# sunhui-3D/3D-PointCloudReconstruction

Hardware: AMD Instinct MI355X
Metric: Chamfer3D fwd+bwd point-pairs/sec @ B=32 N=M=1024; EMD iters/sec (higher is better)
Workload: dtype f32; 1 GPU; Chamfer3D fwd+bwd (+loss sums, +RCCL all-reduce of every step's loss when N>1); batch_per_gpu=32, n_points=1024, m_points=1024, global_batch=32, parallelism=dp1 (batch-sharded), launch=hipgraph (20 steps per graph; N>1 adds each step's all-reduce to the same graph)

## Files before the change

3d-pointcloudreconstruction_amd/csrc/chamfer_filt.hip:

```cpp
#include <type_traits>

#include "pcm_common.h"
#include "pcm_internal.h"
#include "chamfer_loss.h"

namespace {
using namespace pcm_loss;

constexpr float kFiltU16 = 9.5367431640625e-07f;

#ifdef PCM_STAMPS
constexpr int kStampSlots = 1 << 16;
__device__ unsigned long long g_pcm_stamps[kStampSlots * 8];
#define PCM_STAMP(i)                                                                           \
    do {                                                                                       \
        if (threadIdx.x == 0 && blockIdx.x < kStampSlots)                                      \
            g_pcm_stamps[blockIdx.x * 8 + (i)] = __builtin_amdgcn_s_memrealtime();            \
    } while (0)
#define PCM_STAMP2(i)                                                                          \
    do {                                                                                       \
        if (threadIdx.x == 0 && blockIdx.x < kStampSlots / 2)                                  \
            g_pcm_stamps[(kStampSlots / 2 + blockIdx.x) * 8 + (i)] = __builtin_amdgcn_s_memrealtime(); \
    } while (0)
#else
// ... 363 lines not shown
                    if (resident) {
#pragma unroll
                        for (int k = 0; k < CP; ++k) {
                            const int kk = slot(min(k0 + k, nt - 1));
                            const pcm_f4 t4 = sT[kk];
                            tx[k] = t4.x;
                            ty[k] = t4.y;
                            tz[k] = t4.z;
                        }
                    } else {
#pragma unroll
                        for (int k = 0; k < CP; ++k) {
                            const int kk = min(k0 + k, nt - 1);
                            tx[k] = pcm_ld(T + pcm_at(LT, kk, 0));
                            ty[k] = pcm_ld(T + pcm_at(LT, kk, 1));
                            tz[k] = pcm_ld(T + pcm_at(LT, kk, 2));
                        }
                    }
#pragma unroll
                    for (int k = 0; k < CP; ++k) {
                        const float d = pcm_sqd(tx[k] - x, ty[k] - y, tz[k] - z);
                        const bool take = (d < hd) & (k0 + k < nt);
                        hd = take ? d : hd;
                        hk = take ? k0 + k : hk;
                    }
                } else if (part == 0) {
                    unsigned plan = 0;
                    const float thr = fb + e2;
#pragma unroll
                    for (int w = 0; w < W; ++w)
                        plan |= !(vs[w] > thr) ? (1u << (W + w)) : (!(vb[w] > thr) ? (1u << w) : 0u);
                    sPlan[s] = plan;
                    sList[atomicAdd(&sNList, 1)] = s;
                }
            }
            sHD[part][s] = hd;
            sHK[part][s] = hk;
        }
        __syncthreads();
        PCM_STAMP(5);

        const int nl = sNList;
        if (resident) {
            static_assert(C <= 64 && 64 % C == 0 && 64 % W == 0 && (TILE / C) % W == 0,
                          "whole chunks per step; wave w owns the chunks c = w mod W");
            constexpr int kCps = 64 / C;
            unsigned long long wpat = 0;
#pragma unroll
            for (int i = 0; i < 64; i += W) wpat |= 1ull << i;
            const int nch = (nt + C - 1) / C;
            for (int e = wave; e < nl; e += W) {
                const int s = __builtin_amdgcn_readfirstlane(sList[e]);
                const unsigned plan = __builtin_amdgcn_readfirstlane(sPlan[s]);
                int one[W];
#pragma unroll
                for (int w = 0; w < W; ++w) one[w] = __builtin_amdgcn_readfirstlane(sChunk[w][s]);
                float x = rx[0], y = ry[0], z = rz[0];
#pragma unroll
                for (int qq = 1; qq < QPT; ++qq)
                    if ((s >> 6) == qq) { x = rx[qq]; y = ry[qq]; z = rz[qq]; }
                x = __int_as_float(__builtin_amdgcn_readlane(__float_as_int(x), s & 63));
                y = __int_as_float(__builtin_amdgcn_readlane(__float_as_int(y), s & 63));
                z = __int_as_float(__builtin_amdgcn_readlane(__float_as_int(z), s & 63));
                float bd = PCM_INF;
                int bk = 0x7fffffff;
                for (int c0 = 0; c0 < nch; c0 += 64) {
                    unsigned long long M = 0;
#pragma unroll
                    for (int w = 0; w < W; ++w) {
                        if ((plan >> (W + w)) & 1u) M |= wpat << w;
                        else if (((plan >> w) & 1u) && one[w] >= c0 && one[w] < c0 + 64) M |= 1ull << (one[w] - c0);
                    }
                    if (nch - c0 < 64) M &= (1ull << (nch - c0)) - 1ull;
                    while (M) {
                        int ch[kCps];
#pragma unroll
                        for (int j = 0; j < kCps; ++j) {
                            ch[j] = M ? c0 + __builtin_ctzll(M) : -1;
                            M &= M - 1ull;
                        }
                        int c = ch[0];
#pragma unroll
                        for (int j = 1; j < kCps; ++j)
                            if (lane / C == j) c = ch[j];
                        const int k = c * C + (lane & (C - 1));
                        const int sk = slot(min(max(k, 0), nt - 1));
                        const pcm_f4 t4 = sT[sk];
                        const float d = pcm_sqd(t4.x - x, t4.y - y, t4.z - z);
                        if (c >= 0 && k < nt) pcm_lexmin(bd, bk, d, k);
                    }
                }
                pcm_wave_lexmin(bd, bk);
                if (lane == 0) {
                    sD[s] = bd;
                    sK[s] = bk;
                }
            }
            if (nl > 0) __syncthreads();
        }
        for (int e0 = 0; e0 < (resident ? 0 : nl); e0 += kTB) {
            float qx[kTB], qy[kTB], qz[kTB], bd[kTB];
            int bk[kTB];
#pragma unroll
            for (int j = 0; j < kTB; ++j) {
                const int s = sList[min(e0 + j, nl - 1)];
                float x = rx[0], y = ry[0], z = rz[0];
#pragma unroll
                for (int qq = 1; qq < QPT; ++qq)
                    if ((s >> 6) == qq) { x = rx[qq]; y = ry[qq]; z = rz[qq]; }
                qx[j] = __shfl(x, s & 63, 64);
                qy[j] = __shfl(y, s & 63, 64);
                qz[j] = __shfl(z, s & 63, 64);
                bd[j] = PCM_INF;
                bk[j] = 0x7fffffff;
            }
            auto visit = [&](int k, float x, float y, float z) {
#pragma unroll
                for (int j = 0; j < kTB; ++j) {
                    const float d = pcm_sqd(x - qx[j], y - qy[j], z - qz[j]);
                    pcm_lexmin(bd[j], bk[j], d, k);
                }
            };
            {
                constexpr int U = 8;
                for (int k0 = tid; k0 < nt; k0 += U * NT) {
                    float tx[U], ty[U], tz[U];
#pragma unroll
                    for (int u = 0; u < U; ++u) {
                        const int k = min(k0 + u * NT, nt - 1);
                        tx[u] = pcm_ld(T + pcm_at(LT, k, 0));
                        ty[u] = pcm_ld(T + pcm_at(LT, k, 1));
                        tz[u] = pcm_ld(T + pcm_at(LT, k, 2));
                    }
#pragma unroll
                    for (int u = 0; u < U; ++u)
                        if (k0 + u * NT < nt) visit(k0 + u * NT, tx[u], ty[u], tz[u]);
                }
            }
#pragma unroll
            for (int j = 0; j < kTB; ++j) {
#pragma unroll
                for (int o = 32; o > 0; o >>= 1) {
                    const float od = __shfl_xor(bd[j], o, 64);
                    const int ok = __shfl_xor(bk[j], o, 64);
                    pcm_lexmin(bd[j], bk[j], od, ok);
                }
            }
            if (lane == 0) {
#pragma unroll
                for (int j = 0; j < kTB; ++j) {
                    sTD[j * W + wave] = bd[j];
                    sTK[j * W + wave] = bk[j];
                }
            }
            __syncthreads();
            if (tid < kTB && e0 + tid < nl) {
                float d = sTD[tid * W];
                int k = sTK[tid * W];
                for (int w = 1; w < W; ++w) {
                    const float dv = sTD[tid * W + w];
                    const int kv = sTK[tid * W + w];
                    pcm_lexmin(d, k, dv, kv);
                }
                const int s = sList[e0 + tid];
                sD[s] = d;
                sK[s] = k;
            }
            __syncthreads();
        }
        PCM_STAMP(6);
        int kg = 0;
        if (tid < QW && qbase + tid < nq) {
            float d;
            int k;
            if (proven) {
                d = sHD[0][tid];
                k = sHK[0][tid];
#pragma unroll
                for (int p = 1; p < PARTS; ++p) pcm_lexmin(d, k, sHD[p][tid], sHK[p][tid]);
            } else {
                d = sD[tid];
                k = sK[tid];
            }
            my_d = d;
            out_st<kSc1>(D + qbase + tid, d);
            out_st<kSc1>(I + qbase + tid, (int32_t)k);
            if (Gr) __hip_atomic_store(Gr + qbase + tid, tag | (unsigned)k, __ATOMIC_RELAXED, __HIP_MEMORY_SCOPE_AGENT);
            if (Gr4 && !g4x)
                __hip_atomic_store(Gr4 + qbase + tid, gtag4 | (unsigned)k, __ATOMIC_RELAXED, __HIP_MEMORY_SCOPE_AGENT);
            if (kown) *kown = k;
            kg = k;
        }
        if (Gr4 && g4x && tid < QW) {
            const unsigned v = gtag4 | (unsigned)kg;
            const int src = (lane & 15) * 4;
            pcm_u32x4 g;
            g.x = (unsigned)__shfl((int)v, src, 64);
            g.y = (unsigned)__shfl((int)v, src + 1, 64);
            g.z = (unsigned)__shfl((int)v, src + 2, 64);
            g.w = (unsigned)__shfl((int)v, src + 3, 64);
            const int q = qbase + (tid & ~63) + src;
            if (lane < 16 && q < nq) {
                if (q + 3 < nq) {
                    pcm_st_sc1_x4(Gr4 + q, g);
                } else {
                    __hip_atomic_store(Gr4 + q, g.x, __ATOMIC_RELAXED, __HIP_MEMORY_SCOPE_AGENT);
                    if (q + 1 < nq) __hip_atomic_store(Gr4 + q + 1, g.y, __ATOMIC_RELAXED, __HIP_MEMORY_SCOPE_AGENT);
                    if (q + 2 < nq) __hip_atomic_store(Gr4 + q + 2, g.z, __ATOMIC_RELAXED, __HIP_MEMORY_SCOPE_AGENT);
                }
            }
        }
    } else {
        for (int s = tid; s < QW; s += NT) {
            const int qi = qbase + s;
            if (qi >= nq) continue;
            float d;
            int idx;
            pcm_ref_nn_scan(pcm_ld(Q + pcm_at(LQ, qi, 0)), pcm_ld(Q + pcm_at(LQ, qi, 1)),
                            pcm_ld(Q + pcm_at(LQ, qi, 2)), T, nt, d, idx, LT);
            my_d = d;
            out_st<kSc1>(D + qi, d);
            out_st<kSc1>(I + qi, (int32_t)idx);
            if (Gr) __hip_atomic_store(Gr + qi, tag | (unsigned)idx, __ATOMIC_RELAXED, __HIP_MEMORY_SCOPE_AGENT);
            if (Gr4) __hip_atomic_store(Gr4 + qi, gtag4 | (unsigned)idx, __ATOMIC_RELAXED, __HIP_MEMORY_SCOPE_AGENT);
            if (kown) *kown = idx;
        }
    }
    return my_d;
}

constexpr float kFiltU80 = 4.76837158203125e-06f;
constexpr int kMfmaQW = 256, kMfmaNT = 512, kMfmaTile = 1024;
struct MfmaLds {
    static constexpr int kA = kMfmaTile * 48;
    static constexpr int kZ = (3 * 48 + 16) * 16;
    static constexpr int kQB = kMfmaQW * 48;
    static constexpr int kScan = kA + kZ + kQB;
    static constexpr int kTail = 3 * kMfmaTile * 4 + 3 * 4 * kMfmaQW * 4;
    static constexpr int kBytes = kScan > kTail ? kScan : kTail;
};
typedef __bf16 pcm_bf16x8 __attribute__((ext_vector_type(8)));

typedef __bf16 pcm_bf16x2 __attribute__((ext_vector_type(2)));
__device__ __forceinline__ unsigned cvt_bf16x2(float a, float b) {
    return __builtin_bit_cast(unsigned, __builtin_convertvector((pcm_f2){a, b}, pcm_bf16x2));
}
__device__ __forceinline__ float bf_lo(unsigned v) { return __uint_as_float(v << 16); }
__device__ __forceinline__ float bf_hi(unsigned v) { return __uint_as_float(v & 0xffff0000u); }
template <int HL, int HH>
__device__ __forceinline__ unsigned bf_pair(unsigned lo, unsigned hi) {
    constexpr unsigned sel = (HL ? 0x0302u : 0x0100u) | ((HH ? 0x0706u : 0x0504u) << 16);
    return __builtin_amdgcn_perm(hi, lo, sel);
}
[[maybe_unused]] __device__ __forceinline__ void split3x2(float a, float b, unsigned &H, unsigned &M, unsigned &L) {
    H = cvt_bf16x2(a, b);
    const float ra = a - bf_lo(H), rb = b - bf_hi(H);
    M = cvt_bf16x2(ra, rb);
    L = cvt_bf16x2(ra - bf_lo(M), rb - bf_hi(M));
}
[[maybe_unused]] __device__ __forceinline__ int mslot(int p) { return (p & ~63) | ((p + 4 * ((p >> 6) & 7)) & 63); }

template <bool k32>
__device__ __forceinline__ void mfma_fold_step(float &b, float &s, int &c, float bo, float so, int co) {
    auto swap = [](unsigned &x, unsigned &y) {
        if constexpr (k32) {
            const auto r = __builtin_amdgcn_permlane32_swap(x, y, false, false);
            x = r[0];
            y = r[1];
        } else {
            const auto r = __builtin_amdgcn_permlane16_swap(x, y, false, false);
            x = r[0];
            y = r[1];
        }
    };
    unsigned b0 = __float_as_uint(b), b1 = __float_as_uint(bo), s0 = __float_as_uint(s), s1 = __float_as_uint(so);
    unsigned c0 = (unsigned)c, c1 = (unsigned)co;
    swap(b0, b1);
    swap(s0, s1);
    swap(c0, c1);
    const float fb0 = __uint_as_float(b0), fb1 = __uint_as_float(b1);
    const bool better = (fb1 < fb0) | ((fb1 == fb0) & ((int)c1 < (int)c0));
    s = __builtin_fminf(__builtin_fminf(__uint_as_float(s0), __uint_as_float(s1)), better ? fb0 : fb1);
    b = better ? fb1 : fb0;
    c = better ? (int)c1 : (int)c0;
}

template <bool kSc1>
__device__ __forceinline__ float filt_forward_mfma(const float *__restrict__ Q, const float *__restrict__ T, int nq,
                                                   int nt, int qbase, float *__restrict__ D, int32_t *__restrict__ I,
                                                   unsigned char *arena, unsigned long long *__restrict__ Gr = nullptr,
                                                   unsigned long long tag = 0, PcmLay LQ = PcmLay{3, 1},
                                                   PcmLay LT = PcmLay{3, 1}, int *kown = nullptr) {
    constexpr int QW = kMfmaQW, NT = kMfmaNT, W = NT / 64, TILE = kMfmaTile, QPT = QW / 64;
    constexpr int kPer = TILE / NT;
    static_assert(NT == 2 * QW && QPT == 4, "thread = (query slot, part of 2); wave w holds query copy w mod 4");
    uint4 *sA = reinterpret_cast<uint4 *>(arena);
    uint4 *sZ = reinterpret_cast<uint4 *>(arena + MfmaLds::kA);
    uint4 *sQB = reinterpret_cast<uint4 *>(arena + MfmaLds::kA + MfmaLds::kZ);
    auto rowslot = [](int p, int j) { return 48 * (p >> 4) + 16 * j + (p & 15); };
    float(*sT)[TILE] = reinterpret_cast<float(*)[TILE]>(arena);
    float(*sPB)[QW] = reinterpret_cast<float(*)[QW]>(arena + 3 * TILE * 4);
    float(*sPS)[QW] = reinterpret_cast<float(*)[QW]>(arena + 3 * TILE * 4 + 4 * QW * 4);
    int(*sPC)[QW] = reinterpret_cast<int(*)[QW]>(arena + 3 * TILE * 4 + 8 * QW * 4);
    __shared__ float sD[QW];
    __shared__ int sK[QW];
    __shared__ unsigned sPlan[QW];
    __shared__ float sHD[2][QW];
    __shared__ int sHK[2][QW];
    __shared__ float sRmax[W];
    __shared__ int sList[QW];
    __shared__ int sNList;
    __shared__ int sNFm[W];

    const int tid = threadIdx.x, lane = tid & 63;
    const int wave = __builtin_amdgcn_readfirstlane(tid >> 6);

    float rx[QPT], ry[QPT], rz[QPT];
#pragma unroll
    for (int qq = 0; qq < QPT; ++qq) {
        const int qc = min(qbase + qq * 64 + lane, nq - 1);
        rx[qq] = pcm_ld(Q + pcm_at(LQ, qc, 0));
        ry[qq] = pcm_ld(Q + pcm_at(LQ, qc, 1));
        rz[qq] = pcm_ld(Q + pcm_at(LQ, qc, 2));
    }
    float tv[kPer][3];
#pragma unroll
    for (int r = 0; r < kPer; ++r) {
        const int p = min(tid + r * NT, nt - 1);
#pragma unroll
        for (int d = 0; d < 3; ++d) tv[r][d] = pcm_ld(T + pcm_at(LT, p, d));
    }
    bool nonfinite = false;
    float cx = 0.f, cy = 0.f, cz = 0.f;
    int qcnt = 0;
#pragma unroll
    for (int qq = 0; qq < QPT; ++qq) {
        if (qbase + qq * 64 + lane < nq) {
            nonfinite |= !(pcm_finite(rx[qq]) && pcm_finite(ry[qq]) && pcm_finite(rz[qq]));
            cx += rx[qq];
            cy += ry[qq];
            cz += rz[qq];
            ++qcnt;
        }
    }
    if (tid == 0) sNList = 0;
    const float cn = (float)wave_sum_dpp(qcnt);
    const float c0 = wave_sum_dpp(cx) / cn, c1 = wave_sum_dpp(cy) / cn, c2 = wave_sum_dpp(cz) / cn;
    PCM_STAMP(1);
#ifdef PCM_STAMPS
    if (tid == 0 && blockIdx.x < 4096)
        g_pcm_stamps[(8192 + blockIdx.x) * 8 + 1] = __builtin_amdgcn_s_memtime();
#endif

    float qx = rx[0], qy = ry[0], qz = rz[0];
#pragma unroll
    for (int qq = 1; qq < QPT; ++qq)
        if ((wave & (QPT - 1)) == qq) { qx = rx[qq]; qy = ry[qq]; qz = rz[qq]; }
    const float qxc = qx - c0, qyc = qy - c1, qzc = qz - c2;
    {
        unsigned H01, M01, L01, H2, M2, L2;
        split3x2(qxc, qyc, H01, M01, L01);
        split3x2(qzc, 0.f, H2, M2, L2);
        const unsigned one2 = 0x3f803f80u, one0 = 0x00003f80u;
        const int row = tid & (QW - 1);
        if (wave < QPT) {
            sQB[rowslot(row, 0)] = make_uint4(bf_pair<0, 0>(H01, M01), bf_pair<0, 0>(H01, L01), bf_pair<0, 0>(H01, M01),
                                              bf_pair<1, 1>(H01, M01));
            sQB[rowslot(row, 1)] = make_uint4(bf_pair<1, 1>(H01, L01), bf_pair<1, 1>(H01, M01), bf_pair<0, 0>(H2, M2),
                                              bf_pair<0, 0>(H2, L2));
        } else {
            sQB[rowslot(row, 2)] = make_uint4(bf_pair<0, 0>(H2, M2), one2, one0, 0u);
            if (row < MfmaLds::kZ / 16) sZ[row] = make_uint4(0u, 0u, 0u, 0u);
        }
    }
    const int ntp = (nt + 63) & ~63;
    float rt2 = 0.f;
    uint4 rows[kPer][3];
#pragma unroll
    for (int r = 0; r < kPer; ++r) {
        nonfinite |= !(pcm_finite(tv[r][0]) && pcm_finite(tv[r][1]) && pcm_finite(tv[r][2]));
        const float x = tv[r][0] - c0, y = tv[r][1] - c1, z = tv[r][2] - c2;
        const float w = __builtin_fmaf(z, z, __builtin_fmaf(y, y, x * x));
        unsigned H01, M01, L01, H23, M23, L23;
        split3x2(-2.f * x, -2.f * y, H01, M01, L01);
        split3x2(-2.f * z, w, H23, M23, L23);
        rt2 = __builtin_fmaxf(rt2, __builtin_fmaxf(w, bf_hi(H23)));
        const bool pad = tid + r * NT >= nt;
        rows[r][0] = make_uint4(bf_pair<0, 0>(H01, H01), bf_pair<0, 0>(M01, H01), bf_pair<0, 0>(L01, M01),
                                bf_pair<1, 1>(H01, H01));
        rows[r][1] = make_uint4(bf_pair<1, 1>(M01, H01), bf_pair<1, 1>(L01, M01), bf_pair<0, 0>(H23, H23),
                                bf_pair<0, 0>(M23, H23));
        rows[r][2] = make_uint4(bf_pair<0, 0>(L23, M23), bf_pair<1, 1>(H23, M23), L23 >> 16, 0u);
        if (pad) {
            rows[r][0] = make_uint4(0u, 0u, 0u, 0u);
            rows[r][1] = make_uint4(0u, 0u, 0u, 0u);
            rows[r][2] = make_uint4(0u, 0x00007f80u, 0u, 0u);
        }
    }
#pragma unroll
    for (int r = 0; r < kPer; ++r) {
        const int p = tid + r * NT;
        if (p < ntp) {
            sA[rowslot(p, 0)] = rows[r][0];
            sA[rowslot(p, 1)] = rows[r][1];
            sA[rowslot(p, 2)] = rows[r][2];
        }
    }
    {
        const float v = pcm_wave_max_f32(rt2);
        if (lane == 0) sRmax[wave] = v;
    }
    __syncthreads();
    PCM_STAMP(2);

    const int quarter = wave >> 1, half = wave & 1;
    const int g = lane >> 4, col = lane & 15;
    constexpr int QT = QW / 2 / 16;
    const uint4 *pq = g < 3 ? sQB + 48 * half * QT + lane : sZ + col;
    const uint4 *pa = g < 3 ? sA + lane : sZ + col;
    const int tstep = g < 3 ? 48 : 0;
    pcm_bf16x8 bq[QT];
#pragma unroll
    for (int qt = 0; qt < QT; ++qt) bq[qt] = __builtin_bit_cast(pcm_bf16x8, pq[qt * tstep]);
    float best[QT], sec[QT];
    int bchunk[QT];
#pragma unroll
    for (int qt = 0; qt < QT; ++qt) { best[qt] = PCM_INF; sec[qt] = PCM_INF; bchunk[qt] = 0; }
    const int ngroups = ntp >> 6;
    uint4 an[4];
    auto fetch = [&](int gi, int i) { an[i] = pa[4 * gi * tstep + 48 * i]; };
    if (quarter < ngroups) {
#pragma unroll
        for (int i = 0; i < 4; ++i) fetch(quarter, i);
    }
    for (int gi = quarter; gi < ngroups; gi += 4) {
        const int gn = gi + 4 < ngroups ? gi + 4 : gi;
        float mn[QT];
#pragma unroll
        for (int qt = 0; qt < QT; ++qt) mn[qt] = PCM_INF;
#pragma unroll
        for (int i = 0; i < 4; ++i) {
            const pcm_bf16x8 a = __builtin_bit_cast(pcm_bf16x8, an[i]);
            fetch(gn, i);
            __builtin_amdgcn_sched_barrier(0);
#pragma unroll
            for (int qt = 0; qt < QT; ++qt) {
                const pcm_f4 d = __builtin_amdgcn_mfma_f32_16x16x32_bf16(a, bq[qt], pcm_f4{0.f, 0.f, 0.f, 0.f}, 0, 0, 0);
                mn[qt] = __builtin_fminf(__builtin_fminf(mn[qt], d.x), d.y);
                mn[qt] = __builtin_fminf(__builtin_fminf(mn[qt], d.z), d.w);
            }
            __builtin_amdgcn_sched_group_barrier(0x8, 2, 0);
#pragma unroll
            for (int k = 0; k < QT - 2; ++k) {
                __builtin_amdgcn_sched_group_barrier(0x2, 2, 0);
                __builtin_amdgcn_sched_group_barrier(0x8, 1, 0);
            }
        }
        const int cid = 4 * gi + g;
#pragma unroll
        for (int qt = 0; qt < QT; ++qt) {
            sec[qt] = __builtin_amdgcn_fmed3f(mn[qt], best[qt], sec[qt]);
            if (mn[qt] < best[qt]) { best[qt] = mn[qt]; bchunk[qt] = cid; }
        }
    }
    __syncthreads();
    PCM_STAMP(3);
#pragma unroll
    for (int r = 0; r < kPer; ++r) {
        const int p = tid + r * NT;
        if (p < nt) { sT[0][mslot(p)] = tv[r][0]; sT[1][mslot(p)] = tv[r][1]; sT[2][mslot(p)] = tv[r][2]; }
    }
    static_assert(QT == 8, "two halving steps: 8 query tiles -> 2 per lane");
#pragma unroll
    for (int j = 0; j < 4; ++j)
        mfma_fold_step<true>(best[j], sec[j], bchunk[j], best[j + 4], sec[j + 4], bchunk[j + 4]);
#pragma unroll
    for (int j = 0; j < 2; ++j) {
        mfma_fold_step<false>(best[j], sec[j], bchunk[j], best[j + 2], sec[j + 2], bchunk[j + 2]);
        const int s = half * (QW / 2) + (4 * (g >> 1) + 2 * (g & 1) + j) * 16 + col;
        sPB[quarter][s] = best[j];
        sPS[quarter][s] = sec[j];
        sPC[quarter][s] = bchunk[j];
    }
    const int any_nonfinite = pcm_wg_or(nonfinite, sNFm, W);
    PCM_STAMP(4);

    float my_d = 0.f;
    if (!any_nonfinite) {
        const int s = tid & (QW - 1), part = tid / QW;
        bool proven = false;
        {
            float vb[4], vs[4], vr[W];
            int vc[4];
#pragma unroll
            for (int q = 0; q < 4; ++q) {
                vb[q] = sPB[q][s];
                vs[q] = sPS[q][s];
                vc[q] = sPC[q][s];
            }
#pragma unroll
            for (int w = 0; w < W; ++w) vr[w] = sRmax[w];
            __builtin_amdgcn_sched_barrier(0);
            float fb = vb[0], fs = vs[0];
            int fc = vc[0];
#pragma unroll
            for (int q = 1; q < 4; ++q) {
                const bool better = (vb[q] < fb) | ((vb[q] == fb) & (vc[q] < fc));
                fs = __builtin_fminf(__builtin_fminf(fs, vs[q]), better ? fb : vb[q]);
                fb = better ? vb[q] : fb;
                fc = better ? vc[q] : fc;
            }
            float rmax2 = vr[0];
#pragma unroll
            for (int w = 1; w < W; ++w) rmax2 = __builtin_fmaxf(rmax2, vr[w]);
            const float kAbs = 7.888609052210118e-31f;
            const float qn2 = __builtin_fmaf(qzc, qzc, __builtin_fmaf(qyc, qyc, qxc * qxc));
            const float sq = __builtin_amdgcn_sqrtf(qn2);
            const float rr = __builtin_amdgcn_sqrtf(rmax2) + sq;
            const float eR = kFiltU80 * (rr * rr) * 1.001f + kAbs;
            const float db = __builtin_fmaxf((fb + qn2) * 1.0001f + 2.f * eR, 0.f);
            const float rq = 2.f * sq + __builtin_amdgcn_sqrtf(db);
            const float e2 = 2.f * (kFiltU80 * __builtin_fminf(rr * rr, rq * rq) * 1.001f + kAbs);
            proven = (fs - fb) > e2;
            float hd = PCM_INF;
            int hk = 0x7fffffff;
            if (qbase + s < nq) {
                if (proven) {
                    const int k0 = 64 * (fc >> 2) + 32 * part + 4 * (fc & 3);
                    pcm_f4 tx[2], ty[2], tz[2];
#pragma unroll
                    for (int h = 0; h < 2; ++h) {
                        const int o = mslot(k0 + 16 * h);
                        tx[h] = *reinterpret_cast<const pcm_f4 *>(&sT[0][o]);
                        ty[h] = *reinterpret_cast<const pcm_f4 *>(&sT[1][o]);
                        tz[h] = *reinterpret_cast<const pcm_f4 *>(&sT[2][o]);
                    }
#pragma unroll
                    for (int k = 0; k < 8; ++k) {
                        const int kk = k0 + 16 * (k >> 2) + (k & 3);
                        const float d = pcm_sqd(tx[k >> 2][k & 3] - qx, ty[k >> 2][k & 3] - qy, tz[k >> 2][k & 3] - qz);
                        const bool take = (d < hd) & (kk < nt);
                        hd = take ? d : hd;
                        hk = take ? kk : hk;
                    }
                } else if (part == 0) {
                    const float thr = fb + e2;
                    unsigned plan = 0;
#pragma unroll
                    for (int q = 0; q < 4; ++q) plan |= !(vs[q] > thr) ? (1u << q) : (!(vb[q] > thr) ? (16u << q) : 0u);
                    sPlan[s] = plan;
                    sList[atomicAdd(&sNList, 1)] = s;
                }
            }
            sHD[part][s] = hd;
            sHK[part][s] = hk;
        }
        __syncthreads();
        PCM_STAMP(5);
        const int nl = sNList;
        for (int e = wave; e < nl; e += W) {
            const int sq = __builtin_amdgcn_readfirstlane(sList[e]);
            const unsigned plan = __builtin_amdgcn_readfirstlane(sPlan[sq]);
            float x = rx[0], y = ry[0], z = rz[0];
#pragma unroll
            for (int qq = 1; qq < QPT; ++qq)
                if ((sq >> 6) == qq) { x = rx[qq]; y = ry[qq]; z = rz[qq]; }
            x = __int_as_float(__builtin_amdgcn_readlane(__float_as_int(x), sq & 63));
            y = __int_as_float(__builtin_amdgcn_readlane(__float_as_int(y), sq & 63));
            z = __int_as_float(__builtin_amdgcn_readlane(__float_as_int(z), sq & 63));
            float bd = PCM_INF;
            int bk = 0x7fffffff;
            {
                const int pc = sPC[g][sq];
                const int k = 64 * (pc >> 2) + 16 * (col >> 2) + 4 * (pc & 3) + (col & 3);
                const bool on = ((plan >> (4 + g)) & 1u) && k < nt;
                const int ks = mslot(min(k, nt - 1));
                const float d = pcm_sqd(sT[0][ks] - x, sT[1][ks] - y, sT[2][ks] - z);
                if (on) pcm_lexmin(bd, bk, d, k);
            }
            for (int q = 0; q < 4; ++q) {
                if (!((plan >> q) & 1u)) continue;
                float tx[4], ty[4], tz[4];
                int kk[4];
#pragma unroll
                for (int u = 0; u < 4; ++u) {
                    const int k = 64 * (q + 4 * u) + lane;
                    kk[u] = (q + 4 * u < ngroups && k < nt) ? k : -1;
                    const int ks = mslot(min(max(kk[u], 0), nt - 1));
                    tx[u] = sT[0][ks];
                    ty[u] = sT[1][ks];
                    tz[u] = sT[2][ks];
                }
#pragma unroll
                for (int u = 0; u < 4; ++u) {
                    const float d = pcm_sqd(tx[u] - x, ty[u] - y, tz[u] - z);
                    if (kk[u] >= 0) pcm_lexmin(bd, bk, d, kk[u]);
                }
            }
            pcm_wave_lexmin(bd, bk);
            if (lane == 0) {
                sD[sq] = bd;
                sK[sq] = bk;
            }
        }
        if (nl > 0) __syncthreads();
        PCM_STAMP(6);
#ifdef PCM_STAMPS
        if (tid == 0 && blockIdx.x < 4096) g_pcm_stamps[(8192 + blockIdx.x) * 8 + 6] = __builtin_amdgcn_s_memtime();
        if (tid == NT - 1 && blockIdx.x < kStampSlots) {
            unsigned long long full = 0, single = 0;
            for (int e = 0; e < nl; ++e) {
                const unsigned pl = sPlan[sList[e]];
                full += __popc(pl & 15);
                single += __popc((pl >> 4) & 15);
            }
            g_pcm_stamps[blockIdx.x * 8 + 0] = (unsigned long long)nl | (full << 16) | (single << 40);
        }
#endif
        if (tid < QW && qbase + tid < nq) {
            float d;
            int k;
            if (proven) {
                d = sHD[0][tid];
                k = sHK[0][tid];
                pcm_lexmin(d, k, sHD[1][tid], sHK[1][tid]);
            } else {
                d = sD[tid];
                k = sK[tid];
            }
            my_d = d;
            out_st<kSc1>(D + qbase + tid, d);
            out_st<kSc1>(I + qbase + tid, (int32_t)k);
            if (Gr) __hip_atomic_store(Gr + qbase + tid, tag | (unsigned)k, __ATOMIC_RELAXED, __HIP_MEMORY_SCOPE_AGENT);
            if (kown) *kown = k;
        }
    } else {
        for (int s = tid; s < QW; s += NT) {
            const int qi = qbase + s;
            if (qi >= nq) continue;
            float d;
            int idx;
            pcm_ref_nn_scan(pcm_ld(Q + pcm_at(LQ, qi, 0)), pcm_ld(Q + pcm_at(LQ, qi, 1)),
                            pcm_ld(Q + pcm_at(LQ, qi, 2)), T, nt, d, idx, LT);
            my_d = d;
            out_st<kSc1>(D + qi, d);
            out_st<kSc1>(I + qi, (int32_t)idx);
            if (Gr) __hip_atomic_store(Gr + qi, tag | (unsigned)idx, __ATOMIC_RELAXED, __HIP_MEMORY_SCOPE_AGENT);
            if (kown) *kown = idx;
        }
    }
    return my_d;
}

template <typename TIn, int W, int QPT, int C, int TILE, int kLoss>
__global__ __launch_bounds__(64 * W) __attribute__((amdgpu_waves_per_eu(4))) void chamfer_fwd_filt_kernel(
    const TIn *__restrict__ xyz1, const TIn *__restrict__ xyz2, int b, int n, int m,
    float *__restrict__ dist1, float *__restrict__ dist2, int32_t *__restrict__ idx1,
    int32_t *__restrict__ idx2, int nblk1, int nblk2, float *__restrict__ partials,
    unsigned *__restrict__ ticket, float *__restrict__ mean_out) {
    static_assert(kLoss == 0 || kLoss == 3, "filtered forward publishes granules only");
    static_assert(W <= 16, "sRed holds 16 waves");
    constexpr int QW = 64 * QPT;
    __shared__ float sRed[2][16];

    int nprod = (int)gridDim.x;
    unsigned epoch = 0;
    if constexpr (kLoss == 3) {
        nprod -= 1;
        if ((int)blockIdx.x == nprod) {
            poll_loss(b * nblk1, nprod, b, n, m, reinterpret_cast<const unsigned long long *>(partials), ticket,
                      mean_out);
            return;
        }
        epoch = ticket[kEpochWord] + 1u;
    }
    PCM_STAMP(0);
    int batch, blk;
    bool first;
    pcm_split_bm(pcm_xcd_remap((int)blockIdx.x, nprod), nblk1, nblk2, batch, first, blk);
    const int slot = first ? batch * nblk1 + blk : b * nblk1 + batch * nblk2 + blk;
    const TIn *Q = first ? xyz1 + (size_t)batch * n * 3 : xyz2 + (size_t)batch * m * 3;
    const TIn *T = first ? xyz2 + (size_t)batch * m * 3 : xyz1 + (size_t)batch * n * 3;
    float *D = first ? dist1 + (size_t)batch * n : dist2 + (size_t)batch * m;
    int32_t *I = first ? idx1 + (size_t)batch * n : idx2 + (size_t)batch * m;
    const int nq = first ? n : m, nt = first ? m : n;
    const float my_d = filt_forward<TIn, W, QPT, C, TILE, false>(Q, T, nq, nt, blk * QW, D, I,
                                                                 lds_arena<FiltLds<W, QPT, TILE>::kBytes>());
    if constexpr (kLoss == 3) publish_partial<3>(my_d, slot, partials, ticket, sRed, epoch);
#ifdef PCM_STAMPS
    if (threadIdx.x == 0 && blockIdx.x < kStampSlots)
        g_pcm_stamps[blockIdx.x * 8 + 7] = __builtin_amdgcn_s_memrealtime();
#endif
}

template <int W, int QPT, int C, int TILE, int LAY1, int LAY2>
__global__ __launch_bounds__(64 * W) __attribute__((amdgpu_waves_per_eu(4))) void chamfer_fwd_filt_lay_kernel(
    const float *__restrict__ xyz1, const float *__restrict__ xyz2, int b, int n, int m,
    float *__restrict__ dist1, float *__restrict__ dist2, int32_t *__restrict__ idx1,
    int32_t *__restrict__ idx2, int nblk1, int nblk2) {
    constexpr int QW = 64 * QPT;
    int batch, blk;
    bool first;
    pcm_split_bm(pcm_xcd_remap((int)blockIdx.x, (int)gridDim.x), nblk1, nblk2, batch, first, blk);
    const float *X1 = xyz1 + (size_t)batch * n * 3, *X2 = xyz2 + (size_t)batch * m * 3;
    const PcmLay L1 = LAY1 ? PcmLay{1, n} : PcmLay{3, 1}, L2 = LAY2 ? PcmLay{1, m} : PcmLay{3, 1};
    if (first)
        filt_forward<float, W, QPT, C, TILE, false>(X1, X2, n, m, blk * QW, dist1 + (size_t)batch * n,
                                                   idx1 + (size_t)batch * n, lds_arena<FiltLds<W, QPT, TILE>::kBytes>(),
                                                   nullptr, 0, nullptr, nullptr, L1, L2);
    else
        filt_forward<float, W, QPT, C, TILE, false>(X2, X1, m, n, blk * QW, dist2 + (size_t)batch * m,
                                                   idx2 + (size_t)batch * m, lds_arena<FiltLds<W, QPT, TILE>::kBytes>(),
                                                   nullptr, 0, nullptr, nullptr, L2, L1);
}

constexpr int kGradCap = 1024;
constexpr unsigned kG4TagBits = 21;
constexpr unsigned kG4TagMask = (1u << kG4TagBits) - 1u;
static_assert(kGradCap <= 2048, "a 4-byte granule holds an 11-bit index");
constexpr unsigned kGradWaitSpins = 1u << 16;
constexpr int kGradSlots = 8;
constexpr int kGradSlotsMax = 16;
constexpr int kGradBytes = 2 * kGradCap * 12 + 2 * kGradCap * 4 + 2 * kGradCap * kGradSlots * 2;

__device__ __forceinline__ int32_t ld_sc1(const int32_t *p) {
    return __hip_atomic_load(p, __ATOMIC_RELAXED, __HIP_MEMORY_SCOPE_AGENT);
}
__device__ __forceinline__ float ld_sc1(const float *p) {
    return __hip_atomic_load(p, __ATOMIC_RELAXED, __HIP_MEMORY_SCOPE_AGENT);
}

template <typename GetA, typename GetH>
__device__ __forceinline__ void scatter_sum(float &ax, float &ay, float &az, float sx, float sy, float sz,
                                            GetH h, GetA getA, const uint16_t *tab, int cnt) {
    static_assert(kGradSlots == 8 && kGradSlotsMax == 16, "sorting networks for 8 and 16 ids");
    if (cnt > kGradSlots) {
        int f[16];
        const uint4 r0 = *reinterpret_cast<const uint4 *>(tab);
        const uint4 r1 = *reinterpret_cast<const uint4 *>(tab + 8);
        const unsigned wv[8] = {r0.x, r0.y, r0.z, r0.w, r1.x, r1.y, r1.z, r1.w};
#pragma unroll
        for (int u = 0; u < 16; ++u) {
            const int t = (int)((wv[u >> 1] >> (16 * (u & 1))) & 0xffffu);
            f[u] = u < cnt ? t : 0x7fffffff;
        }
#pragma unroll
        for (int rd = 0; rd < 16; ++rd)
#pragma unroll
            for (int i = rd & 1; i + 1 < 16; i += 2) {
                const int lo = min(f[i], f[i + 1]), hi = max(f[i], f[i + 1]);
                f[i] = lo;
                f[i + 1] = hi;
            }
        for (int u = 0; u < cnt; ++u) {
            float tx, ty, tz;
            getA(f[u], tx, ty, tz);
            const float hu = h(f[u]);
            ax = __fadd_rn(ax, -__fmul_rn(hu, __fsub_rn(tx, sx)));
            ay = __fadd_rn(ay, -__fmul_rn(hu, __fsub_rn(ty, sy)));
            az = __fadd_rn(az, -__fmul_rn(hu, __fsub_rn(tz, sz)));
        }
        return;
    }
    int e[8];
    const uint4 row = *reinterpret_cast<const uint4 *>(tab);
    const unsigned w[4] = {row.x, row.y, row.z, row.w};
#pragma unroll
    for (int u = 0; u < 8; ++u) {
        const int t = (int)((w[u >> 1] >> (16 * (u & 1))) & 0xffffu);
        e[u] = u < cnt ? t : 0x7fffffff;
    }
    auto cas = [&](int i, int j) {
        const int lo = min(e[i], e[j]), hi = max(e[i], e[j]);
        e[i] = lo;
        e[j] = hi;
    };
    cas(0, 1); cas(2, 3); cas(4, 5); cas(6, 7); cas(0, 2); cas(1, 3); cas(4, 6); cas(5, 7); cas(1, 2);
    cas(5, 6); cas(0, 4); cas(3, 7); cas(1, 5); cas(2, 6); cas(1, 4); cas(3, 6); cas(2, 4); cas(3, 5);
    cas(3, 4);
    auto add = [&](float hu, float tx, float ty, float tz) {
        ax = __fadd_rn(ax, -__fmul_rn(hu, __fsub_rn(tx, sx)));
        ay = __fadd_rn(ay, -__fmul_rn(hu, __fsub_rn(ty, sy)));
        az = __fadd_rn(az, -__fmul_rn(hu, __fsub_rn(tz, sz)));
    };
    float gx[4], gy[4], gz[4], gh[4];
#pragma unroll
    for (int u = 0; u < 4; ++u) {
        const int su = u < cnt ? e[u] : 0;
        getA(su, gx[u], gy[u], gz[u]);
        gh[u] = h(su);
    }
#pragma unroll
    for (int u = 0; u < 4; ++u) {
        const bool on = u < cnt;
        const float nx = __fadd_rn(ax, -__fmul_rn(gh[u], __fsub_rn(gx[u], sx)));
        const float ny = __fadd_rn(ay, -__fmul_rn(gh[u], __fsub_rn(gy[u], sy)));
        const float nz = __fadd_rn(az, -__fmul_rn(gh[u], __fsub_rn(gz[u], sz)));
        ax = on ? nx : ax;
        ay = on ? ny : ay;
        az = on ? nz : az;
    }
    for (int u = 4; u < cnt; ++u) {
        float tx, ty, tz;
        getA(e[u], tx, ty, tz);
        add(h(e[u]), tx, ty, tz);
    }
}

constexpr int kBwdSlotsT = 256;
constexpr int kBwdSlotsMax = 2048;

struct PcmRescale {
    const float *gl = nullptr;
    const float *used = nullptr;
    float *next = nullptr;
    float inv1 = 0.f, inv2 = 0.f;
};

__device__ __forceinline__ void slots_task(int task, int ntasks, const float *__restrict__ xyz1,
                                           const float *__restrict__ xyz2, int n, int m,
                                           const float *__restrict__ gd1, const float *__restrict__ gd2,
                                           const int32_t *__restrict__ idx1, const int32_t *__restrict__ idx2,
                                           float *__restrict__ grad1, float *__restrict__ grad2, int nblk1, int nblk2,
                                           int lay1, int lay2, PcmGdStr GS, bool rescale, float rs1, float rs2) {
    constexpr int NT = kBwdSlotsT;
    __shared__ __attribute__((aligned(16))) float sO[3 * kBwdSlotsMax];
    __shared__ __attribute__((aligned(16))) float sG[kBwdSlotsMax];
    __shared__ __attribute__((aligned(16))) int sK[kBwdSlotsMax];
    __shared__ int cnt[NT];
    __shared__ __attribute__((aligned(16))) uint16_t tab[NT * kGradSlotsMax];
    const int tid = threadIdx.x;
    const int wave = tid >> 6;
    int batch, blk;
    bool first;
    pcm_split_bm(pcm_xcd_remap(task, ntasks), nblk1, nblk2, batch, first, blk);
    const int ns = first ? n : m, no = first ? m : n;
    const float rs_self = first ? rs1 : rs2, rs_other = first ? rs2 : rs1;
    const float *self = first ? xyz1 + (size_t)batch * n * 3 : xyz2 + (size_t)batch * m * 3;
    const float *other = first ? xyz2 + (size_t)batch * m * 3 : xyz1 + (size_t)batch * n * 3;
    const int gbs = first ? (GS.bs1 < 0 ? n : GS.bs1) : (GS.bs2 < 0 ? m : GS.bs2);
    const int gbo = first ? (GS.bs2 < 0 ? m : GS.bs2) : (GS.bs1 < 0 ? n : GS.bs1);
    const int gps = rescale ? 0 : (first ? GS.ps1 : GS.ps2), gpo = rescale ? 0 : (first ? GS.ps2 : GS.ps1);
    const float *gds = (first ? gd1 : gd2) + (size_t)batch * gbs;
    const float *gdo = (first ? gd2 : gd1) + (size_t)batch * gbo;
    const int32_t *ids = (first ? idx1 + (size_t)batch * n : idx2 + (size_t)batch * m);
    const int32_t *ido = (first ? idx2 + (size_t)batch * m : idx1 + (size_t)batch * n);
    float *grad = first ? grad1 + (size_t)batch * n * 3 : grad2 + (size_t)batch * m * 3;
    const PcmLay LS = first ? pcm_lay(lay1, n) : pcm_lay(lay2, m);
    const PcmLay LO = first ? pcm_lay(lay2, m) : pcm_lay(lay1, n);
    const int t0 = blk * NT;
    const int T = min(NT, ns - t0);

    pcm_dma_to_lds(sK, ido, 4 * no, wave, NT / 64);
    pcm_dma_to_lds(sO, other, 12 * no, wave, NT / 64);
    float hconst = 0.f;
    if (rescale)
        hconst = __fmul_rn(rs_other, 2.f);
    else if (gpo == 1)
        pcm_dma_to_lds(sG, gdo, 4 * no, wave, NT / 64);
    else if (gpo == 0)
        hconst = __fmul_rn(gdo[0], 2.f);
    else
        for (int j = tid; j < no; j += NT) sG[j] = gdo[(size_t)j * gpo];
    const int i = t0 + tid;
    const bool own = tid < T;
    float sx = 0.f, sy = 0.f, sz = 0.f, gself = 0.f;
    int kself = 0;
    if (own) {
        sx = self[pcm_at(LS, i, 0)];
        sy = self[pcm_at(LS, i, 1)];
        sz = self[pcm_at(LS, i, 2)];
        kself = ids[i];
// ... 1011 lines not shown
```

Measured before the change: 5283 billion point-pairs/s.

## Software-pipeline MFMA results with lagged min-fold and stage raw queries in LDS

Flattens the MFMA distance loop into a single 32-step sequence with a rotating set of four result registers. Each min-fold is delayed by three steps, and the best/second-best update for the previous chunk is interleaved into the next chunk's MFMAs, so the MFMA latency is hidden without manual sched_group_barrier hints. Separately, the raw query coordinates are written to spare LDS at the end of the arena, so the refinement loop reads them directly instead of using a select chain plus readlane. The change costs extra registers for the rotated accumulators, adds LDS traffic, and makes chunk-id tracking across iterations more delicate.

Result: faster. 5509 billion point-pairs/s (median of 6 runs) (+4.3%).

```diff
diff --git a/3d-pointcloudreconstruction_amd/csrc/chamfer_filt.hip b/3d-pointcloudreconstruction_amd/csrc/chamfer_filt.hip
--- a/3d-pointcloudreconstruction_amd/csrc/chamfer_filt.hip
+++ b/3d-pointcloudreconstruction_amd/csrc/chamfer_filt.hip
@@ -689,6 +689,8 @@
     float(*sPB)[QW] = reinterpret_cast<float(*)[QW]>(arena + 3 * TILE * 4);
     float(*sPS)[QW] = reinterpret_cast<float(*)[QW]>(arena + 3 * TILE * 4 + 4 * QW * 4);
     int(*sPC)[QW] = reinterpret_cast<int(*)[QW]>(arena + 3 * TILE * 4 + 8 * QW * 4);
+    float(*sQR)[QW] = reinterpret_cast<float(*)[QW]>(arena + MfmaLds::kTail);
+    static_assert(MfmaLds::kTail + 3 * QW * 4 <= MfmaLds::kBytes, "raw queries fit the arena behind the partials");
     __shared__ float sD[QW];
     __shared__ int sK[QW];
     __shared__ unsigned sPlan[QW];
@@ -820,36 +822,42 @@
 #pragma unroll
         for (int i = 0; i < 4; ++i) fetch(quarter, i);
     }
+    constexpr int kRot = 4, kLag = 3;
+    float mn[QT];
+#pragma unroll
+    for (int qt = 0; qt < QT; ++qt) mn[qt] = PCM_INF;
+    pcm_f4 d[kRot];
+#pragma unroll
+    for (int r = 0; r < kRot; ++r) d[r] = pcm_f4{PCM_INF, PCM_INF, PCM_INF, PCM_INF};
+    int cid = 0;
+    auto fold = [&](int k, bool first) {
+        const pcm_f4 r = d[k % kRot];
+        mn[k % QT] = __builtin_fminf(__builtin_fminf(first ? PCM_INF : mn[k % QT], r.x), r.y);
+        mn[k % QT] = __builtin_fminf(__builtin_fminf(mn[k % QT], r.z), r.w);
+    };
+    auto update = [&](int qt) {
+        sec[qt] = __builtin_amdgcn_fmed3f(mn[qt], best[qt], sec[qt]);
+        if (mn[qt] < best[qt]) { best[qt] = mn[qt]; bchunk[qt] = cid; }
+    };
     for (int gi = quarter; gi < ngroups; gi += 4) {
         const int gn = gi + 4 < ngroups ? gi + 4 : gi;
-        float mn[QT];
-#pragma unroll
-        for (int qt = 0; qt < QT; ++qt) mn[qt] = PCM_INF;
-#pragma unroll
-        for (int i = 0; i < 4; ++i) {
-            const pcm_bf16x8 a = __builtin_bit_cast(pcm_bf16x8, an[i]);
-            fetch(gn, i);
+#pragma unroll
+        for (int k = 0; k < 4 * QT; ++k) {
+            d[k % kRot] = __builtin_amdgcn_mfma_f32_16x16x32_bf16(__builtin_bit_cast(pcm_bf16x8, an[k / QT]), bq[k % QT],
+                                                                  pcm_f4{0.f, 0.f, 0.f, 0.f}, 0, 0, 0);
+            if (k % QT == QT - 1) fetch(gn, k / QT);
             __builtin_amdgcn_sched_barrier(0);
-#pragma unroll
-            for (int qt = 0; qt < QT; ++qt) {
-                const pcm_f4 d = __builtin_amdgcn_mfma_f32_16x16x32_bf16(a, bq[qt], pcm_f4{0.f, 0.f, 0.f, 0.f}, 0, 0, 0);
-                mn[qt] = __builtin_fminf(__builtin_fminf(mn[qt], d.x), d.y);
-                mn[qt] = __builtin_fminf(__builtin_fminf(mn[qt], d.z), d.w);
-            }
-            __builtin_amdgcn_sched_group_barrier(0x8, 2, 0);
-#pragma unroll
-            for (int k = 0; k < QT - 2; ++k) {
-                __builtin_amdgcn_sched_group_barrier(0x2, 2, 0);
-                __builtin_amdgcn_sched_group_barrier(0x8, 1, 0);
-            }
-        }
-        const int cid = 4 * gi + g;
-#pragma unroll
-        for (int qt = 0; qt < QT; ++qt) {
-            sec[qt] = __builtin_amdgcn_fmed3f(mn[qt], best[qt], sec[qt]);
-            if (mn[qt] < best[qt]) { best[qt] = mn[qt]; bchunk[qt] = cid; }
-        }
-    }
+            if (k < kLag) fold(4 * QT - kLag + k, false);
+            else fold(k - kLag, k - kLag < QT);
+            if (k < QT) update(k);
+            __builtin_amdgcn_sched_barrier(0);
+        }
+        cid = 4 * gi + g;
+    }
+#pragma unroll
+    for (int k = 4 * QT - kLag; k < 4 * QT; ++k) fold(k, false);
+#pragma unroll
+    for (int qt = 0; qt < QT; ++qt) update(qt);
     __syncthreads();
     PCM_STAMP(3);
 #pragma unroll
@@ -857,6 +865,7 @@
         const int p = tid + r * NT;
         if (p < nt) { sT[0][mslot(p)] = tv[r][0]; sT[1][mslot(p)] = tv[r][1]; sT[2][mslot(p)] = tv[r][2]; }
     }
+    if (tid < QW) { sQR[0][tid] = qx; sQR[1][tid] = qy; sQR[2][tid] = qz; }
     static_assert(QT == 8, "two halving steps: 8 query tiles -> 2 per lane");
 #pragma unroll
     for (int j = 0; j < 4; ++j)
@@ -948,13 +957,7 @@
         for (int e = wave; e < nl; e += W) {
             const int sq = __builtin_amdgcn_readfirstlane(sList[e]);
             const unsigned plan = __builtin_amdgcn_readfirstlane(sPlan[sq]);
-            float x = rx[0], y = ry[0], z = rz[0];
-#pragma unroll
-            for (int qq = 1; qq < QPT; ++qq)
-                if ((sq >> 6) == qq) { x = rx[qq]; y = ry[qq]; z = rz[qq]; }
-            x = __int_as_float(__builtin_amdgcn_readlane(__float_as_int(x), sq & 63));
-            y = __int_as_float(__builtin_amdgcn_readlane(__float_as_int(y), sq & 63));
-            z = __int_as_float(__builtin_amdgcn_readlane(__float_as_int(z), sq & 63));
+            const float x = sQR[0][sq], y = sQR[1][sq], z = sQR[2][sq];
             float bd = PCM_INF;
             int bk = 0x7fffffff;
             {
```
